# zjucsxxd/hdr2yuv

Measured on AMD Instinct MI355X. Metric: Mpixels/s, 4K RGB->YUV420 PQ convert path (in-memory, HBM-resident), higher is better.
Workload: dtype f32+f64

## Files before the change

hdr2yuv_amd/csrc/h2y_api.hip:

```cpp
#include <hip/hip_runtime.h>

#include <cstdarg>
#include <cstdio>
#include <cstdlib>
#include <algorithm>
#include <cstring>
#include <new>
#include <string>
#include <vector>

#include "../../include/hdr2yuv_hip.h"
#include "h2y_kernels.h"
#include "h2y_math.h"
#include "h2y_walk.h"

#include <zlib.h>

using namespace h2y;

namespace {

thread_local std::string g_err;

struct clip_limits {
// ... 79 lines not shown
    std::vector<double> bal_bwork;
    std::vector<uint32_t> range_slot[2];
    bool slot_busy[2] = {false, false};
    uint32_t *d_unit_rows = nullptr, *h_unit_rows = nullptr;
    size_t unit_rows_cap = 0;
    std::vector<uint32_t> dev_unit_rows;
    bool ffb_pending = false;
    double ffb_work[8] = {0, 0, 0, 0, 0, 0, 0, 0};
    frame_stats *d_fstats = nullptr, *h_fstats = nullptr;
    frame_stats *m_fstats = nullptr;
    frame_stats *fs_out = nullptr;
    assumed_stats *d_assumed = nullptr, *h_assumed = nullptr;
    assumed_stats dev_assumed;
    bool dev_assumed_ok = false;
    h2y_desc p_desc;
    int p_n = 0;
    bool p_check = false;
    bool was_t1 = false;
    std::vector<frame_io> p_frames;
    hipEvent_t ev_done = nullptr;
    hipEvent_t ev[kMaxEvents][2];
    int n_ev = 0;
};

struct h2y_ctx {
    int device = 0;
    batch_state bs[2];
    batch_state *b = &bs[0];
    int q_head = 0, q_count = 0;
    int n_cu = 0;
    hipStream_t own_stream = nullptr, stream = nullptr;
    hipStream_t fir_stream = nullptr;
    hipEvent_t ev_fused[2] = {nullptr, nullptr}, ev_fir[2] = {nullptr, nullptr};
    bool fir_used[2] = {false, false};
    void *d_table = nullptr;
    void *d_table1 = nullptr;
    void *d_table_ext = nullptr;
    void *d_tfn[H2Y_TFN_COUNT] = {};
    void *d_tfn_ext[H2Y_TFN_COUNT] = {};
    float *d_lut16 = nullptr;
    bool bal_have = false;
    double bal_speed[8] = {1, 1, 1, 1, 1, 1, 1, 1};
    std::vector<double> bal_bspeed;
    int bal_bgrid = 0, bal_bgroups = 0;
    bool ffb_have = false;
    double ffb_speed[8] = {1, 1, 1, 1, 1, 1, 1, 1};
    int t1_skip = 0, t1_skip_len = 0;
    bool cur_skip_t1 = false;
    bool opt_t1 = true;
    bool opt_t1_steer = true;
    int opt_groups = 0;
    bool opt_cols8 = true;
    int opt_bal_mode = 0;
    int opt_tail = 2;
    bool opt_bal_blocks = true;
    uint32_t opt_bal_mask = 0xFFu;
    double opt_bal_rho = 1.0;
    int opt_fir = 0;
    int opt_fir_sync = -1;
    double fir_flag_share = 0.0;
    uint16_t *d_tmp = nullptr;
    size_t tmp_cap = 0;
    uint16_t *d_lin = nullptr;
    void *d_tab = nullptr, *h_tab = nullptr;
    size_t d_tab_cap = 0, h_tab_cap = 0;
    cmp_partial *d_cmp_part = nullptr;
    size_t cmp_part_cap = 0;
    h2y_compare_stats *d_cmp_stats = nullptr;
    size_t cmp_stats_cap = 0;
    char *d_hist = nullptr;
    size_t hist_cap = 0;
    int64_t *d_ssim_part = nullptr;
    size_t ssim_part_cap = 0;
    h2y_ssim_stats *d_ssim_stats = nullptr;
    size_t ssim_stats_cap = 0;
    assumed_stats *d_light_as = nullptr;
    size_t light_as_cap = 0;
    light_acc *d_light_acc = nullptr;
    size_t light_acc_cap = 0;

    void *d_in = nullptr;
    size_t in_cap = 0;
    uint16_t *d_out = nullptr;
    size_t out_cap = 0;
    bool have_hint = false;
    int hint_kind = -1;
    int32_t hint_floor[3] = {0, 0, 0}, hint_ceil[3] = {0, 0, 0};
    struct stream_slot {
        char *h_in = nullptr;
        uint16_t *h_out = nullptr;
        char *d_in = nullptr;
        uint16_t *d_out = nullptr;
        hipEvent_t ev_h2d = nullptr, ev_conv = nullptr, ev_done = nullptr;
        int state = 0;
        char *h_ref = nullptr, *d_ref = nullptr;
        h2y_compare_stats *h_stats = nullptr;
        bool ref_lent = false;
        char *d_hist = nullptr;
        h2y_histogram_stats *h_hist_stats = nullptr;
        uint32_t *h_hist_bins = nullptr;
        h2y_ssim_stats *d_ssim = nullptr, *h_ssim = nullptr;
        light_acc *d_light = nullptr, *h_light = nullptr;
    };
    std::vector<stream_slot> ss;
    hipStream_t s_h2d = nullptr, s_d2h = nullptr;
    h2y_desc s_desc;
// ... 562 lines not shown
        for (int i = 0; i < nf; i++) {
            frame_io io = frames[f0 + i];
            if (out_kind == H2Y_OUT_444TMP) {
                io.tmp_cb = ctx->d_tmp + ((size_t)half * fir_sub + i) * tmp_stride;
                io.tmp_cr = io.tmp_cb + npix;
            } else if (yuvp2) {
                io.yuv = io.out;
                io.out = ctx->d_tmp + ((size_t)half * fir_sub + i) * tmp_stride;
                io.tmp_cr = nullptr;
            }
            const size_t idx = (size_t)ctx->slot_base + f0 + i;
            on_device = on_device && memcmp(&ctx->b->dev_frames[idx], &io, sizeof io) == 0;
            ctx->b->h_frames[idx] = io;
        }
        if (!on_device) {
            HIP_TRY(ctx, hipMemcpyAsync(ctx->b->d_frames + ctx->slot_base + f0, ctx->b->h_frames + ctx->slot_base + f0, nf * sizeof(frame_io), hipMemcpyHostToDevice,
                                        ctx->stream));
            for (int i = 0; i < nf; i++) ctx->b->dev_frames[(size_t)ctx->slot_base + f0 + i] = ctx->b->h_frames[(size_t)ctx->slot_base + f0 + i];
        }
        const int grid = grid_for(ctx, var, (uint64_t)g.chunks * nf);
        const int waves = h2y_fused_threads(var) / 64;
        int groups = 1;
        if (h2y_fused_grouped(var))
            for (int ng = groups_cap(ctx, g.tiles, grid); ng > 1; ng >>= 1)
                if (nf % ng == 0 && grid % ng == 0) {
                    groups = ng;
                    break;
                }
        if (nf / groups > kMaxFramesPerLaunch) return fail(ctx, H2Y_EINVAL, "internal: %d frames in %d groups exceed the per-group bound", nf, groups);
        int rc = ensure(ctx, ctx->b->d_partial, ctx->b->partial_cap, (size_t)nf * grid * waves * 6 * sizeof(float));
        if (rc) return rc;
        const bool t1 = var.pipe == 4 || var.pipe == 5;
        if (t1) {
            rc = ensure(ctx, ctx->b->d_redo, ctx->b->redo_cap, (size_t)nf * grid * waves * sizeof(uint32_t));
            if (rc) return rc;
        }
        const bool approx = var.pipe == 4;
        if (approx) {
            const size_t need = (size_t)(nf > 64 ? nf : 64) * sizeof(uint32_t);
            if (ctx->b->low_cap < need) {
                rc = ensure(ctx, ctx->b->d_low, ctx->b->low_cap, need);
                if (rc) return rc;
                HIP_TRY(ctx, hipMemsetAsync(ctx->b->d_low, 0, need, ctx->stream));
            }
        }
        if (check) ctx->b->approx_min = approx;
        const bool xcd_layout = h2y_fused_grouped(var) && grid % (8 * groups) == 0;
        const uint32_t *d_slice_ranges = nullptr;
        uint32_t range_stride = 0;
        bool tail_on = false;
        uint32_t tail_slices = 0;
        std::vector<double> bwork;
        double work[8] = {1, 1, 1, 1, 1, 1, 1, 1};
        if (xcd_layout && ctx->opt_bal_mode != 1) {
            const uint32_t G = (uint32_t)grid / (uint32_t)groups, nslices = (g.tiles + 63u) / 64u;
            double sp[8], mean = 0.0;
            for (int x = 0; x < 8; x++) {
                sp[x] = ctx->opt_bal_mode == 2 ? (((ctx->opt_bal_mask >> x) & 1u) ? ctx->opt_bal_rho : 1.0) : (ctx->bal_have ? ctx->bal_speed[x] : 1.0);
                mean += sp[x] / 8.0;
            }
            for (int x = 0; x < 8; x++) work[x] = sp[x] / mean;
            const bool per_block = ctx->opt_bal_mode == 0 && ctx->opt_bal_blocks && ctx->bal_bgrid == grid && ctx->bal_bgroups == groups &&
                                   (int)ctx->bal_bspeed.size() == grid && (size_t)groups * (G + 1u) <= kRangeWords;
            std::vector<uint32_t> r(per_block ? (size_t)groups * (G + 1u) : (size_t)G + 1u);
            bwork.assign((size_t)grid, 1.0);
            if (per_block) {
                std::vector<double> w(G);
                for (uint32_t gi = 0; gi < (uint32_t)groups; gi++) {
                    for (uint32_t i = 0; i < G; i++) w[i] = ctx->bal_bspeed[walk_block_of(gi, i, (uint32_t)groups)];
                    slice_ranges_w(w.data(), G, nslices, r.data() + (size_t)gi * (G + 1u));
                }
                range_stride = G + 1u;
            } else slice_ranges(sp, G, nslices, r.data());
            const int per_group = nf / groups;
            tail_on = t1 && ctx->opt_tail != 2 && nf % groups == 0 && per_group >= (ctx->opt_tail == 1 ? 2 : kTailMinFrames) && groups <= 16 &&

                      (uint64_t)(nslices / H2Y_TAIL_CHUNK + 96u) * 2u <= 64ull * G && G >= 8u;
            tail_slices = nslices;
            for (uint32_t gi = 0; gi < (uint32_t)groups; gi++) {
                const uint32_t *rg = r.data() + (size_t)(per_block ? gi : 0u) * (G + 1u);
                for (uint32_t i = 0; i < G; i++) bwork[walk_block_of(gi, i, (uint32_t)groups)] = (double)(rg[i + 1] - rg[i]) * (double)G / (double)nslices;
            }
            if (!ctx->b->h_ranges) {
                HIP_TRY(ctx, hipHostMalloc((void **)&ctx->b->h_ranges, 2 * kRangeWords * sizeof(uint32_t), hipHostMallocMapped));
                HIP_TRY(ctx, hipHostGetDevicePointer((void **)&ctx->b->hd_ranges, ctx->b->h_ranges, 0));
                HIP_TRY(ctx, hipHostMalloc((void **)&ctx->b->h_btime, 1024 * sizeof(float), hipHostMallocMapped));
                HIP_TRY(ctx, hipHostGetDevicePointer((void **)&ctx->b->hd_btime, ctx->b->h_btime, 0));
            }
            if (r.size() > kRangeWords) return fail(ctx, H2Y_EINVAL, "internal: %zu slice ranges", r.size());
            if (sub == 0 && !ctx->streaming) ctx->b->slot_busy[0] = ctx->b->slot_busy[1] = false;
            int slot = -1;
            for (int k = 0; k < 2 && slot < 0; k++)
                if (ctx->b->range_slot[k] == r) slot = k;
            if (slot < 0) {
                for (int k = 0; k < 2 && slot < 0; k++)
                    if (!ctx->b->slot_busy[k]) slot = k;
                if (slot < 0) {
                    HIP_TRY(ctx, hipStreamSynchronize(ctx->stream));
                    ctx->b->slot_busy[0] = ctx->b->slot_busy[1] = false;
                    slot = 0;
                }
                memcpy(ctx->b->h_ranges + (size_t)slot * kRangeWords, r.data(), r.size() * sizeof(uint32_t));
                ctx->b->range_slot[slot] = r;
            }
            ctx->b->slot_busy[slot] = true;
            d_slice_ranges = ctx->b->hd_ranges + (size_t)slot * kRangeWords;
        }
        const bool clocks = xcd_layout && time_it;
        if (clocks) {
            const size_t need = (size_t)2 * grid * sizeof(unsigned long long);
            if (ctx->b->clock_cap < need) {
                rc = ensure(ctx, ctx->b->d_clock, ctx->b->clock_cap, need);
                if (rc) return rc;
                HIP_TRY(ctx, hipMemsetAsync(ctx->b->d_clock, 0, need, ctx->stream));
            }
        }
        fused_args a;
        a.xcd_layout = xcd_layout ? 1u : 0u;
        a.block_clock = clocks ? ctx->b->d_clock : nullptr;
        a.slice_ranges = d_slice_ranges;
        a.range_stride = range_stride;
        a.tail_ctr = nullptr;
        a.tail_slices = 0;
        if (tail_on && d_slice_ranges) {
            if (!ctx->b->d_tail) {
                HIP_TRY(ctx, hipMalloc((void **)&ctx->b->d_tail, 16 * H2Y_TAIL_WORDS * sizeof(uint32_t)));
                HIP_TRY(ctx, hipMemsetAsync(ctx->b->d_tail, 0, 16 * H2Y_TAIL_WORDS * sizeof(uint32_t), ctx->stream));
            }
            a.tail_ctr = ctx->b->d_tail;
            a.tail_slices = tail_slices;
        }
        a.redo_count = t1 ? ctx->b->d_redo : nullptr;
        a.low_flag = approx ? ctx->b->d_low : nullptr;
        a.frames = ctx->b->d_frames + ctx->slot_base + f0;
        a.n_frames = nf;
        a.width = d->width;
        a.height = d->height;
        a.wq = g.wq;
        a.wq_magic = g.wq_magic;
        a.tiles_per_frame = g.tiles;
        a.chunks_per_frame = g.chunks;
        a.groups = (uint32_t)groups;
        a.table = ctx->d_table;
        a.table_src = a.table_dst = nullptr;
        a.lut16 = ctx->d_lut16;
        a.table1 = ctx->d_table1;
        a.sn = sn;
        a.partial = ctx->b->d_partial;
        a.assumed = d_assumed;
        a.pp = pp;
        if (pp.convert_transfer == 2 && !var.narrow && (var.pipe == 0 || var.pipe == 7)) {
            static const int kSrcFn[4] = {H2Y_TFN_NONE, H2Y_TFN_PQ_F, H2Y_TFN_RHO_H, H2Y_TFN_G24};
            static const int kDstFn[4] = {H2Y_TFN_NONE, H2Y_TFN_PQ_R, H2Y_TFN_RHO_R, H2Y_TFN_G24INV};
            const int sf = kSrcFn[pp.src_tf], df = kDstFn[pp.dst_tf];
            int rc2 = ensure_tfn(ctx, sf);
            if (!rc2) rc2 = ensure_tfn(ctx, df);
            if (rc2) return rc2;
            a.pp.src_fn = sf;
            a.pp.dst_fn = df;
            a.table_src = sf ? ctx->d_tfn[sf] : nullptr;
            a.table_dst = df ? ctx->d_tfn[df] : nullptr;
            a.pp.tf_ext[0] = sf ? ctx->d_tfn_ext[sf] : nullptr;
            a.pp.tf_ext[1] = df ? ctx->d_tfn_ext[df] : nullptr;
        }
        a.tiles_magic = g.tiles > 1 ? (uint32_t)(0x100000000ull / g.tiles) : 0xFFFFFFFFu;
        const bool ev = time_it && ctx->b->n_ev < kMaxEvents;
        if (ev) {
            HIP_TRY(ctx, hipEventRecord(ctx->b->ev[ctx->b->n_ev][0], ctx->stream));
            ctx->last_name = h2y_fused_name(var);
            static const char *const kIn[] = {"F32", "F16", "U16"}, *const kOut[] = {"420BOX", "444", "444TMP"};
            static const char *const kPipe[] = {"RUNTIME", "PQ_IDENT", "PQ_NORM", "LUT16", "PQ_IDENT", "PQ_NORM", "NONE", "TFN"};
            const char *mode = var.mode == H2Y_MODE_YCBCR ? "YCBCR" : var.mode == H2Y_MODE_YDZDX ? "YDZDX" : var.mode == H2Y_MODE_IDENTITY ? "IDENTITY"
                             : var.mode == H2Y_MODE_YUVP2 ? "YUVP2" : "YPQRS";
            char buf[192];
            snprintf(buf, sizeof buf, "%s<%s,%s,%s,%s%s>%s groups=%d xcd=%d%s", ctx->last_name, kIn[var.in_kind], kOut[var.out_kind], mode,
                     kPipe[var.pipe], var.cols8 ? ",COLS8" : "", out_kind == H2Y_OUT_444TMP ? "+k_fir420" : yuvp2 ? (d->chroma_resampler_type ? "+k_yuvp2_420<FIR>" : "+k_yuvp2_420<BOX>") : "", groups, xcd_layout ? 1 : 0,
                     a.tail_ctr ? " tail=1" : "");
            ctx->last_variant = buf;
        }
        HIP_TRY(ctx, h2y_launch_fused(var, grid, ctx->stream, a));
        if (ev) {
            HIP_TRY(ctx, hipEventRecord(ctx->b->ev[ctx->b->n_ev][1], ctx->stream));
            ctx->b->n_ev++;
        }
        final_args fa;
        fa.partial = ctx->b->d_partial;
        fa.nblk = grid / groups * waves;
        fa.redo_count = t1 ? ctx->b->d_redo : nullptr;
        fa.low_flag = approx ? ctx->b->d_low : nullptr;
        fa.out = ctx->b->fs_out + fstats_offset + f0;
        fa.is_u16 = d->in_sample_type == H2Y_SAMPLE_U16;
        fa.src_bit_depth = d->src_bit_depth;
        fa.check = check ? 1 : 0;
        fa.assumed = d_assumed;
        fa.publish = nullptr;
        fa.block_clock = clocks ? ctx->b->d_clock : nullptr;
        fa.grid = grid;
        static_assert(sizeof(frame_stats) >= 8 * sizeof(float), "the XCD run times ride in one frame_stats entry");
        fa.xcd_time = reinterpret_cast<float *>(ctx->b->fs_out + fstats_offset + n);
        fa.tail_ctr = a.tail_ctr;
        fa.tail_n = groups * (int)H2Y_TAIL_WORDS;
        fa.block_time = clocks && d_slice_ranges && ctx->b->fs_out == ctx->b->m_fstats ? ctx->b->hd_btime : nullptr;
        HIP_TRY(ctx, h2y_launch_stats_final(nf, ctx->stream, fa));
        if (clocks) {
            ctx->b->bal_slot = fstats_offset + n;
            ctx->b->bal_pending = true;
            for (int x = 0; x < 8; x++) ctx->b->bal_work[x] = work[x];
            ctx->b->bal_grid = fa.block_time ? grid : 0;
            ctx->b->bal_groups = groups;
            ctx->b->bal_bwork = bwork;
        }
        if (yuvp2) {
            HIP_TRY(ctx, hipEventRecord(ctx->ev_fused[half], ctx->stream));
            HIP_TRY(ctx, hipStreamWaitEvent(ctx->fir_stream, ctx->ev_fused[half], 0));
            yuvp2_args ya;
            ya.frames = ctx->b->d_frames + ctx->slot_base + f0;
            ya.n_frames = nf;
            ya.width = d->width;
            ya.height = d->height;
            ya.lin = ctx->d_lin;
            ya.fir_max = pp.fir_max;
            derive_params(d, &ya.pp, false);
            HIP_TRY(ctx, h2y_launch_yuvp2_420(d->chroma_resampler_type == 1, ctx->fir_stream, ya));
            HIP_TRY(ctx, hipEventRecord(ctx->ev_fir[half], ctx->fir_stream));
            ctx->fir_used[half] = true;
        }
        if (out_kind == H2Y_OUT_444TMP) {
            HIP_TRY(ctx, hipEventRecord(ctx->ev_fused[half], ctx->stream));
            HIP_TRY(ctx, hipStreamWaitEvent(ctx->fir_stream, ctx->ev_fused[half], 0));
            fir_args fr;
// ... 214 lines not shown
    if (e != hipSuccess || ndev < 1)
        return fail(nullptr, H2Y_EHIP, "no HIP device (%s): this library has no CPU path", hipGetErrorString(e));
    if (device < 0 || device >= ndev) return fail(nullptr, H2Y_EINVAL, "device %d out of range (have %d)", device, ndev);
    h2y_ctx *ctx = new (std::nothrow) h2y_ctx();
    if (!ctx) return fail(nullptr, H2Y_ENOMEM, "out of host memory");
    const int rc = ctx_init(ctx, device);
    if (rc) {
        h2y_ctx_destroy(ctx);
        return rc;
    }
    *out = ctx;
    return H2Y_OK;
}

int h2y_ctx_set_option(h2y_ctx *ctx, const char *name, const char *value)
{
    if (!ctx) return fail(nullptr, H2Y_EINVAL, "null ctx");
    if (!name || !value) return fail(ctx, H2Y_EINVAL, "null option name or value");
    if ((ctx->q_count > 0) || ctx->streaming) return fail(ctx, H2Y_EINVAL, "a batch is pending or a stream is open");
    if (!strcmp(name, "t1")) {
        ctx->opt_t1 = value[0] != '0';
        ctx->opt_t1_steer = strcmp(value, "always") != 0;
    }
    else if (!strcmp(name, "cols8")) ctx->opt_cols8 = value[0] != '0';
    else if (!strcmp(name, "firsync")) {
        int v = atoi(value), p = 1;
        if (!strcmp(value, "auto")) v = -1;
        else if (v < 0) return fail(ctx, H2Y_EINVAL, "firsync must be >= 0 or \"auto\"");
        while (2 * p <= v && p < 1024) p *= 2;
        ctx->opt_fir_sync = v > 0 ? p : v;
    } else if (!strcmp(name, "groups")) {
        int v = atoi(value), p = 1;
        if (v < 0) return fail(ctx, H2Y_EINVAL, "groups must be >= 0");
        while (2 * p <= v && p < 64) p *= 2;
        ctx->opt_groups = v ? p : 0;
    } else if (!strcmp(name, "balance")) {
        if (!strcmp(value, "adaptive")) { ctx->opt_bal_mode = 0; ctx->opt_bal_blocks = true; }
        else if (!strcmp(value, "xcd")) { ctx->opt_bal_mode = 0; ctx->opt_bal_blocks = false; }
        else if (!strcmp(value, "off")) ctx->opt_bal_mode = 1;
        else {
            char *end = nullptr;
            const unsigned long mm = strtoul(value, &end, 0);
            const double r = (end && *end == ',') ? atof(end + 1) : 0.0;
            if (!(mm & 0xFFu) || (mm & 0xFFu) == 0xFFu || !(r > 1.0)) return fail(ctx, H2Y_EINVAL, "balance: want adaptive, xcd, off or <mask>,<ratio > 1>");
            ctx->opt_bal_mode = 2;
            ctx->opt_bal_mask = (uint32_t)(mm & 0xFFu);
            ctx->opt_bal_rho = r;
        }
    } else if (!strcmp(name, "tail")) {
        if (!strcmp(value, "auto")) ctx->opt_tail = 0;
        else if (!strcmp(value, "on")) ctx->opt_tail = 1;
        else if (!strcmp(value, "off")) ctx->opt_tail = 2;
        else return fail(ctx, H2Y_EINVAL, "tail: want auto, on or off");
    } else if (!strcmp(name, "fir")) {
        if (!strcmp(value, "auto")) ctx->opt_fir = 0;
        else if (!strcmp(value, "twopass")) ctx->opt_fir = 1;
        else if (!strcmp(value, "fused")) ctx->opt_fir = 2;
        else return fail(ctx, H2Y_EINVAL, "fir: want auto, twopass or fused");
    } else return fail(ctx, H2Y_EINVAL, "unknown option '%s'", name);
    return H2Y_OK;
}

void h2y_ctx_destroy(h2y_ctx *ctx)
{
    if (!ctx) return;
    (void)hipSetDevice(ctx->device);
    if (ctx->stream) (void)hipStreamSynchronize(ctx->stream);
    if (ctx->streaming) (void)h2y_stream_close(ctx);
    for (batch_state &b : ctx->bs) {
        for (int i = 0; i < kMaxEvents; i++) {
            if (b.ev[i][0]) (void)hipEventDestroy(b.ev[i][0]);
            if (b.ev[i][1]) (void)hipEventDestroy(b.ev[i][1]);
        }
        if (b.ev_done) (void)hipEventDestroy(b.ev_done);
        (void)hipFree(b.d_frames);
        (void)hipHostFree(b.h_frames);
        (void)hipFree(b.d_partial);
        (void)hipFree(b.d_redo);
        (void)hipFree(b.d_low);
        (void)hipFree(b.d_clock);
        (void)hipHostFree(b.h_ranges);
        (void)hipHostFree(b.h_btime);
        (void)hipFree(b.d_tail);
        (void)hipFree(b.d_unit_rows);
        (void)hipHostFree(b.h_unit_rows);
        (void)hipFree(b.d_fstats);
        (void)hipHostFree(b.h_fstats);
        (void)hipFree(b.d_assumed);
        (void)hipHostFree(b.h_assumed);
    }
    (void)hipFree(ctx->d_table);
    for (void *t : ctx->d_tfn) (void)hipFree(t);
    for (int fn = 0; fn < H2Y_TFN_COUNT; fn++)
        if (ctx->d_tfn_ext[fn] && ctx->d_tfn_ext[fn] != ctx->d_table_ext) (void)hipFree(ctx->d_tfn_ext[fn]);
    (void)hipFree(ctx->d_lut16);
    (void)hipFree(ctx->d_table1);
    (void)hipFree(ctx->d_table_ext);
    (void)hipFree(ctx->d_tmp);
    (void)hipFree(ctx->d_lin);
    (void)hipFree(ctx->d_tab);
    (void)hipHostFree(ctx->h_tab);
    (void)hipFree(ctx->d_cmp_part);
    (void)hipFree(ctx->d_cmp_stats);
    (void)hipFree(ctx->d_hist);
    (void)hipFree(ctx->d_ssim_part);
    (void)hipFree(ctx->d_ssim_stats);
// ... 2564 lines not shown
```

hdr2yuv_amd/csrc/h2y_kernels.h:

```cpp
#ifndef H2Y_KERNELS_H
#define H2Y_KERNELS_H

#include <hip/hip_runtime.h>
#include <stdint.h>

#include "h2y_math.h"

#ifndef H2Y_FUSED_THREADS
#define H2Y_FUSED_THREADS 512
#endif
#ifndef H2Y_FUSED_MINWAVES
#define H2Y_FUSED_MINWAVES 4
#endif

#ifndef H2Y_LOOP_THREADS
#define H2Y_LOOP_THREADS 1024
#endif

#define H2Y_LUT16_N 16384

enum { H2Y_IN_F32 = 0, H2Y_IN_F16 = 1, H2Y_IN_U16 = 2 };
enum { H2Y_OUT_420BOX = 0, H2Y_OUT_444 = 1, H2Y_OUT_444TMP = 2 };

struct frame_io {
    const void *in[3];
    uint16_t *out;
    union {
        uint16_t *tmp_cb;
        uint16_t *yuv;
    };
    uint16_t *tmp_cr;
};

struct frame_stats {
    float mm[6];
    int32_t floor_[3];
    int32_t ceil_[3];
    int32_t mismatch;
    uint32_t redone;
};

struct assumed_stats {
    int32_t floor_[3];
    int32_t ceil_[3];
};

struct fused_args {
    const frame_io *frames;
    int n_frames;
    uint32_t width, height;
    uint32_t wq;
    uint32_t wq_magic;
    uint32_t tiles_per_frame;
    uint32_t chunks_per_frame;
    uint32_t groups;
    uint32_t xcd_layout;
    unsigned long long *block_clock;
    const uint32_t *slice_ranges;
    uint32_t *tail_ctr = nullptr;
    uint32_t tail_slices = 0;
    uint32_t range_stride = 0;
    const void *table;
    const void *table_src, *table_dst;
    const float *lut16;
    const void *table1;
    h2y::t1_sens sn;
    uint32_t tiles_magic;
    float *partial;
    uint32_t *redo_count;
    uint32_t *low_flag;
    const assumed_stats *assumed;
    h2y::pix_params pp;
};

struct fused_variant {
    int in_kind, out_kind, mode;
    int pipe;
    bool narrow;
    bool even_h;
    bool t1_ok = false;
    bool cols8 = false;
};

struct stats_args {
    const void *in[3];
    size_t npix;
    int vec_ok;
    float *partial;
};

struct final_args {
    const float *partial;
    const uint32_t *redo_count;
    uint32_t *low_flag;
    int nblk;
    frame_stats *out;
    int is_u16, src_bit_depth;
    int check;
    const assumed_stats *assumed;
    assumed_stats *publish;
    unsigned long long *block_clock;
    int grid;
    float *xcd_time;
    float *block_time = nullptr;
    uint32_t *tail_ctr = nullptr;
    int tail_n = 0;
};

struct fir_args {
    const frame_io *frames;
    int n_frames;
    const uint16_t *src_cb, *src_cr;
    uint16_t *dst_cb, *dst_cr;
// ... 197 lines not shown
```

hdr2yuv_amd/csrc/h2y_kernels.hip:

```cpp
#include <hip/hip_runtime.h>
#include <stdint.h>
#include <string.h>
#include <stdio.h>

#include "h2y_math.h"
#include "h2y_kernels.h"
#include "h2y_walk.h"
#include "h2y_device.h"

struct tile_pos {
    uint32_t tt;
    uint32_t q0, q1;
    bool row1;
};
__device__ __forceinline__ tile_pos tile_locate(uint32_t tt, uint32_t W, uint32_t H, uint32_t WQ, uint32_t magic)
{
    tile_pos t;
    uint32_t cg;
    (void)udiv_magic(tt, WQ, magic, cg);
    t.tt = tt;
    t.q0 = 2u * tt - cg;
    t.row1 = tt < WQ * (H >> 1);
    t.q1 = t.row1 ? t.q0 + WQ : t.q0;
    return t;
// ... 510 lines not shown
    const frame_io *frames;
    uint32_t *low_flag;
    uint32_t width, height, wq, wq_magic, tiles_per_frame, tiles_magic;
};
template <int IN_KIND, int OUT_KIND, int MODE, int PIPE>
__device__ __forceinline__ void redo_pass(const redo_ctx *rc, const pix_params *spp, const pq_recA *sA, const uint32_t *list,
                                                    uint32_t first, uint32_t cnt)
{
    const uint32_t lane = threadIdx.x & (WAVE - 1);
    if (lane >= cnt) return;
    const pq_recB *sB = reinterpret_cast<const pq_recB *>(sA + H2Y_PQ_NREC);
    uint32_t tt;
    const uint32_t f = udiv_magic(list[first + lane], rc->tiles_per_frame, rc->tiles_magic, tt);
    const frame_io io = rc->frames[f];
    const tile_pos t = tile_locate(tt, rc->width, rc->height, rc->wq, rc->wq_magic);
    tile_in v;
    tile_load<IN_KIND>(io, t, v);
    if (PIPE == H2Y_PIPE_PQ_IDENT && rc->low_flag) {
        float lo = min3f(min3f(v.g0[0], v.g0[1], v.g0[2]), min3f(v.g0[3], v.g1[0], v.g1[1]), min3f(v.g1[2], v.g1[3], v.b0[0]));
        lo = min3f(lo, min3f(v.b0[1], v.b0[2], v.b0[3]), min3f(v.b1[0], v.b1[1], v.b1[2]));
        lo = min3f(lo, min3f(v.b1[3], v.r0[0], v.r0[1]), min3f(v.r0[2], v.r0[3], v.r1[0]));
        lo = min3f(lo, min3f(v.r1[1], v.r1[2], v.r1[3]), lo);
        if (lo <= -1.0f) rc->low_flag[f] = 1u;
    }
    tile_out o;
    tile_exact<OUT_KIND, MODE, PIPE>(*spp, spp, sA, sB, v, o);
    tile_store<OUT_KIND>(io, t, rc->width, rc->height, o);
}

#ifdef H2Y_BLOCK_TIMES
__device__ unsigned long long g_block_times[2 * 1024];
void h2y_dump_block_times(const char *path)
{
    static unsigned long long h[2 * 1024];
    if (hipMemcpyFromSymbol(h, HIP_SYMBOL(g_block_times), sizeof h) != hipSuccess) return;
    FILE *f = fopen(path, "w");
    if (!f) return;
    for (int i = 0; i < 1024; i++) fprintf(f, "%d %llu %llu\n", i, h[2 * i], h[2 * i + 1]);
    fclose(f);
}
#endif
template <int IN_KIND, int OUT_KIND, int MODE, int PIPE>
__global__ __launch_bounds__(H2Y_T1_THREADS) void k_fused_t1(fused_args a)
{
#ifdef H2Y_BLOCK_TIMES
    if (threadIdx.x == 0) g_block_times[2 * blockIdx.x] = wall_clock64();
#endif
    __shared__ pq_rec1 s_t1[H2Y_T1_NREC];
    __shared__ pq_recA s_t2[2 * H2Y_PQ_NREC];
    __shared__ uint32_t s_redo[H2Y_T1_THREADS / WAVE][H2Y_REDO_CAP];
    __shared__ pix_params s_pp;
    __shared__ redo_ctx s_rc;
    __shared__ uint32_t s_claim[H2Y_CLAIM_FRAMES], s_scratch[WAVE];
    __shared__ uint32_t s_tq[H2Y_TAIL_QLEN + 3], s_tbounds[1];
    {
        stage16<H2Y_T1_THREADS, H2Y_T1_NREC>(a.table1, s_t1);
        stage_table<H2Y_T1_THREADS>(a.table, s_t2);
        if (threadIdx.x < H2Y_CLAIM_FRAMES) s_claim[threadIdx.x] = 0u;
        if (threadIdx.x < H2Y_TAIL_QLEN) s_tq[threadIdx.x] = 0xFFFFFFFFu;
        if (threadIdx.x == 0) {
            s_tq[H2Y_TAIL_QLEN] = (blockIdx.x * 37u) & (H2Y_TAIL_PARTS - 1u);
            s_tq[H2Y_TAIL_QLEN + 1] = 0u;
            s_tq[H2Y_TAIL_QLEN + 2] = 0u;
        }
        if (a.tail_ctr && threadIdx.x == 0) s_tbounds[0] = a.tail_slices;
    }
    const pix_params pp = with_assumed(a.pp, a.assumed);
    t1_sens sn = a.sn;
    asm volatile("" : "+v"(sn.a_lo), "+v"(sn.a_hi));
    if (threadIdx.x == 0) {
        s_pp = pp;
        s_rc.frames = a.frames;
        s_rc.low_flag = a.low_flag;
        s_rc.width = a.width; s_rc.height = a.height; s_rc.wq = a.wq; s_rc.wq_magic = a.wq_magic;
        s_rc.tiles_per_frame = a.tiles_per_frame; s_rc.tiles_magic = a.tiles_magic;
    }
    __syncthreads();
    __shared__ uint32_t s_black[3];
    if (threadIdx.x == 0) {
        const pq_recB *sB2 = reinterpret_cast<const pq_recB *>(s_t2 + H2Y_PQ_NREC);
        const float G0 = norm1<PIPE>(pp, 0, 0.0f), B0 = norm1<PIPE>(pp, 1, 0.0f), R0 = norm1<PIPE>(pp, 2, 0.0f);
        uint32_t y, cb, cr;
        if (pixel_fast<MODE, PIPE>(pp, s_t2, sB2, G0, B0, R0, y, cb, cr)) {
            const ycc k = pixel_careful<MODE>(&s_pp, G0, B0, R0);
            y = k.y; cb = k.cb; cr = k.cr;
        }
        s_black[0] = y; s_black[1] = cb - pp.half_m1; s_black[2] = cr - pp.half_m1;
    }
    __syncthreads();

    block_clock_start(a);
    const uint32_t W = a.width, H = a.height;
    const uint32_t lane = threadIdx.x & (WAVE - 1), wave = threadIdx.x / WAVE;
    const pq_recB *const sB2 = reinterpret_cast<const pq_recB *>(s_t2 + H2Y_PQ_NREC);
    uint32_t *const my_list = s_redo[wave];
    uint32_t n_redo = 0;
    tile_in v;
    tile_pos t_cur;
    bool have = false;
    typedef in_traits<IN_KIND> IN;
    frame_walk fw;
    uint32_t fo = 0;
    uint32_t tick = 0;
    bool hold = false;
    uint32_t dyn_carry = 0, dyn_t0_next = 0;
    walk_init(fw, a);
    typedef const __attribute__((address_space(4))) fused_args *args_ptr;
    args_ptr ap = (args_ptr)__builtin_amdgcn_kernarg_segment_ptr();
    const uint32_t grp = (uint32_t)fw.f;
    uint32_t r_first, r_count;
    const bool ranged = block_range(a, fw, r_first, r_count);
    constexpr uint32_t kTqNone = 0xFFFFFFFFu, kTqEmpty = 0xFFFFFFFEu;
    volatile uint32_t *const tq = s_tq;
    uint32_t *const tail_ctr = a.tail_ctr ? a.tail_ctr + grp * H2Y_TAIL_WORDS : nullptr;
    auto draw_chunk = [&](uint32_t c) {
        tail_state ts;
        ts.part = tq[H2Y_TAIL_QLEN];
        ts.tried = tq[H2Y_TAIL_QLEN + 1];
        const uint32_t n_slices = s_tbounds[0];
        uint32_t got = kTqEmpty;
        uint32_t known[2] = {0u, 0u};
        while (!ts.done()) {
            if ((known[ts.part >> 5] >> (ts.part & 31u)) & 1u) { ts.skip(); continue; }
            uint32_t cv = 0u;
            if (lane == 0) cv = __hip_atomic_fetch_add(tail_ctr + ts.part, 1u, __ATOMIC_RELAXED, __HIP_MEMORY_SCOPE_AGENT);
            uint32_t first, count;
            if (ts.take(n_slices, __builtin_amdgcn_readfirstlane(cv), &first, &count)) {
                got = first | (count << 24);
                break;
            }
            uint32_t k0 = 0u, k1 = 0u;
            if (lane == 0) {
                k0 = __hip_atomic_fetch_or(tail_ctr + H2Y_TAIL_PARTS + (ts.part >> 5), 1u << (ts.part & 31u), __ATOMIC_RELAXED, __HIP_MEMORY_SCOPE_AGENT);
                k1 = __hip_atomic_load(tail_ctr + H2Y_TAIL_PARTS + ((ts.part >> 5) ^ 1u), __ATOMIC_RELAXED, __HIP_MEMORY_SCOPE_AGENT);
            }
            known[ts.part >> 5] = __builtin_amdgcn_readfirstlane(k0) | (1u << (ts.part & 31u));
            known[(ts.part >> 5) ^ 1u] = __builtin_amdgcn_readfirstlane(k1);
            ts.skip();
        }
        if (lane == 0) {
            tq[H2Y_TAIL_QLEN] = ts.part;
            tq[H2Y_TAIL_QLEN + 1] = ts.tried;
            asm volatile("" ::: "memory");
            tq[c] = got;
        }
    };
    auto dyn_tile0 = [&](uint32_t tk, uint32_t &tile0) -> bool {
        const uint32_t c = tk / H2Y_TAIL_CHUNK, idx = tk % H2Y_TAIL_CHUNK;
        if (c >= H2Y_TAIL_QLEN) return false;
        if (tk == 0u) draw_chunk(0u);
        uint32_t e;
        while ((e = tq[c]) == kTqNone) __builtin_amdgcn_s_sleep(1);
        asm volatile("" ::: "memory");
        if (idx == 0u && c + 1u < H2Y_TAIL_QLEN) {
            if (e == kTqEmpty) { if (lane == 0) tq[c + 1u] = kTqEmpty; }
            else draw_chunk(c + 1u);
        }
        if (e == kTqEmpty) return false;
        const uint32_t cnt = e >> 24;
        tile0 = ((e & 0xFFFFFFu) + (idx < cnt ? idx : cnt - 1u)) * WAVE;
        return true;
    };
    for (; fw.f < fw.n_frames; fw.advance(), fo++) {
        const int f = fw.f;
        const bool dyn = tail_ctr != nullptr && !fw.has_next();
        const bool dyn_n = tail_ctr != nullptr && fw.has_next() && f + 2 * (int)fw.NG >= fw.n_frames;
        uint32_t dyn_t0 = 0;
        asm volatile("" : "+s"(ap));
        const frame_io *const frames = ap->frames;
        const frame_io io = uniform_io(frames + f);
        typedef const __attribute__((address_space(4))) frame_io *frame_cptr;
        const frame_cptr io_next_p = (frame_cptr)(uintptr_t)(frames + (fw.has_next() ? f + (int)fw.NG : f));
        mm6 mm;
        mm.reset();
        const uint32_t id_base = (uint32_t)f * a.tiles_per_frame;
        uint32_t flagged_f = 0;
        uint32_t flagged_px = 0;
        wave_deal deal, deal_n;
        if (ranged) {
            deal.set_range(r_first, r_count);
            deal_n.set_range(r_first, r_count);
        } else {
            deal.set(fw, fw.k0, H2Y_T1_THREADS / WAVE);
            deal_n.set(fw, fw.k0_n, H2Y_T1_THREADS / WAVE);
        }
        if (dyn) {
            if (!hold) {
                tick = wave_claim(&s_tq[H2Y_TAIL_QLEN + 2], s_scratch, true);
                hold = dyn_tile0(tick, dyn_t0);
            } else dyn_t0 = dyn_carry;
        } else if (!hold) {
            tick = wave_claim(&s_claim[fo], s_scratch, true);
            hold = tick < deal.total;
        }
        bool more = hold;
        while (more) {
            if (!have) {
                t_cur = tile_locate(umin32((dyn ? dyn_t0 : deal.tile0<H2Y_T1_THREADS>(tick)) + lane, a.tiles_per_frame - 1u), W, H, a.wq, a.wq_magic);
                tile_load<IN_KIND>(io, t_cur, v);
            }
#pragma unroll
            for (int j = 0; j < 4; j++)
                asm volatile("" ::"v"(v.g0[j]), "v"(v.b0[j]), "v"(v.r0[j]), "v"(v.g1[j]), "v"(v.b1[j]), "v"(v.r1[j]));
            do {
                const uint32_t tt = (dyn ? dyn_t0 : deal.tile0<H2Y_T1_THREADS>(tick)) + lane;
                tile_pos t = t_cur;
                t.row1 = true;
                const void *src[3];
                int kind;
                uint32_t tick2;
                tile_pos t2;
                const uint32_t n1v = wave_claim_issue(dyn ? &s_tq[H2Y_TAIL_QLEN + 2] : &s_claim[fo], s_scratch);

                tile_in nx;
                {
                        {
                            const uint32_t n1 = __builtin_amdgcn_readfirstlane(n1v);
                            uint32_t tt2;
                            if (__builtin_expect(dyn, 0)) {
                                uint32_t t0n = 0;
                                const bool same = dyn_tile0(n1, t0n);
                                kind = same ? 1 : 0;
                                tick2 = same ? n1 : tick;
                                tt2 = same ? t0n : dyn_t0;
                                dyn_t0_next = tt2;
                            } else {
                            const bool same = n1 < deal.total;
                            if (__builtin_expect(same, 1)) {
                                kind = 1;
                                tick2 = n1;
                                tt2 = deal.tile0<H2Y_T1_THREADS>(n1);
                            } else {
                                const bool try_next = fw.has_next();
                                bool nextf;
                                uint32_t n2, t0n = 0;
                                if (dyn_n) {
                                    n2 = wave_claim(&s_tq[H2Y_TAIL_QLEN + 2], s_scratch, true);
                                    nextf = dyn_tile0(n2, t0n);
                                    dyn_carry = t0n;
                                } else {
                                    n2 = wave_claim(&s_claim[(fo + 1u) & (H2Y_CLAIM_FRAMES - 1u)], s_scratch, try_next);
                                    nextf = try_next && n2 < deal_n.total;
                                    if (nextf) t0n = deal_n.tile0<H2Y_T1_THREADS>(n2);
                                }
                                kind = nextf ? 2 : 0;
                                tick2 = nextf ? n2 : tick;
                                tt2 = nextf ? t0n : deal.tile0<H2Y_T1_THREADS>(tick);
                            }
                            }
                            kind = __builtin_amdgcn_readfirstlane(kind);
                            tick2 = __builtin_amdgcn_readfirstlane(tick2);
                            tt2 = __builtin_amdgcn_readfirstlane(tt2);
                            hold = have = kind != 0;
#pragma unroll
                            for (int c = 0; c < 3; c++) src[c] = io.in[c];
                            if (__builtin_expect(kind == 2, 0)) {
#pragma unroll
                                for (int c = 0; c < 3; c++) src[c] = io_next_p->in[c];
                            }
                            t2 = tile_locate(umin32(tt2 + lane, a.tiles_per_frame - 1u), W, H, a.wq, a.wq_magic);
                        }
                    IN::load4q(src[0], t2.q0, nx.g0);
                    IN::load4q(src[1], t2.q0, nx.b0);
                    IN::load4q(src[2], t2.q0, nx.r0);
                    IN::load4q(src[0], t2.q1, nx.g1);
                    IN::load4q(src[1], t2.q1, nx.b1);
                    IN::load4q(src[2], t2.q1, nx.r1);
                    __builtin_amdgcn_sched_barrier(0);
                }
                tile_out o;
                uint32_t sb[2], sr[2];
                uint64_t redo_m = 0;
#pragma unroll
                for (int row = 0; row < 2; row++) {
                    const float(&gv)[4] = row ? v.g1 : v.g0;
                    const float(&bv)[4] = row ? v.b1 : v.b0;
                    const float(&rv)[4] = row ? v.r1 : v.r0;
#ifdef H2Y_EXP_NOSTATS
                    if (false) {
#else
                    if (PIPE == H2Y_PIPE_PQ_IDENT) {
#endif
                        if (row == 0) { mm.add2(0, gv[0], gv[1]); mm.add2(1, bv[0], bv[1]); mm.add2(2, rv[0], rv[1]); }
                        else { mm.add2_max(0, gv[0], gv[1]); mm.add2_max(1, bv[0], bv[1]); mm.add2_max(2, rv[0], rv[1]); }
                        mm.add2_max(0, gv[2], gv[3]); mm.add2_max(1, bv[2], bv[3]); mm.add2_max(2, rv[2], rv[3]);
                    } else {
#ifndef H2Y_EXP_NOSTATS
                        mm.add2(0, gv[0], gv[1]); mm.add2(0, gv[2], gv[3]);
                        mm.add2(1, bv[0], bv[1]); mm.add2(1, bv[2], bv[3]);
                        mm.add2(2, rv[0], rv[1]); mm.add2(2, rv[2], rv[3]);
#endif
                    }
                    uint32_t Y[4], Cb[4], Cr[4];
                    bool zrow = false;
                    if (__builtin_expect(__builtin_amdgcn_ballot_w64(f2bits(gv[0]) != 0u) == 0, 0)) {
                        const uint32_t z = (f2bits(gv[1]) | f2bits(gv[2]) | f2bits(gv[3])) | (f2bits(bv[0]) | f2bits(bv[1]) | f2bits(bv[2])) |
                                           (f2bits(bv[3]) | f2bits(rv[0]) | f2bits(rv[1])) | (f2bits(rv[2]) | f2bits(rv[3]));
                        zrow = __builtin_amdgcn_ballot_w64(z != 0u) == 0;
                    }
                    if (zrow) {
                        const uint32_t y0 = s_black[0], cb0 = s_black[1], cr0 = s_black[2];
#pragma unroll
                        for (int col = 0; col < 4; col++) { Y[col] = y0; Cb[col] = cb0; Cr[col] = cr0; }
                    } else
#pragma unroll
                    for (int col = 0; col < 4; col++) {
#ifdef H2Y_EXP_NOCOMPUTE
                        Y[col] = f2bits(gv[col]) >> 20; Cb[col] = f2bits(bv[col]) >> 20; Cr[col] = f2bits(rv[col]) >> 20;
                        continue;
#endif
#ifdef H2Y_HALF_COMPUTE
// ... 798 lines not shown
```

hdr2yuv_amd/csrc/h2y_walk.h:

```cpp
#ifndef H2Y_WALK_H
#define H2Y_WALK_H
#include "h2y_math.h"

namespace h2y {

struct walk_args {
    uint32_t groups, xcd_layout, chunks_per_frame;
    int n_frames;
};

struct frame_walk {
    uint32_t G, NG, bi;
    uint32_t cpf, mod, gb;
    int f, n_frames;
    uint32_t k0, k0_n;

    H2Y_FN uint32_t wrap(uint32_t x) const { return x >= G ? x - G : x; }
    H2Y_FN void set_firsts()
    {
        k0 = wrap(bi + G - gb);
        k0_n = wrap(bi + G - wrap(gb + mod));
    }
    H2Y_FN void init(const walk_args &a, uint32_t b , uint32_t grid )
    {
// ... 33 lines not shown
        return same ? 1 : next ? 2 : 0;
    }
    H2Y_FN uint32_t count(uint32_t k) const { return k < cpf ? (cpf - 1u - k) / G + 1u : 0u; }
    H2Y_FN size_t slot() const { return (size_t)f * G + bi; }
};

inline void slice_ranges_w(const double *w , uint32_t G, uint32_t n_slices, uint32_t *r)
{
    double tot = 0.0;
    for (uint32_t i = 0; i < G; i++) tot += w[i];
    double cum = 0.0;
    for (uint32_t i = 0; i <= G; i++) {
        r[i] = i == G ? n_slices : (uint32_t)(cum / tot * (double)n_slices + 0.5);
        if (i < G) cum += w[i];
    }
}
inline void slice_ranges(const double speed[8], uint32_t G, uint32_t n_slices, uint32_t *r)
{
    double w[1024];
    for (uint32_t i = 0; i < G && i < 1024u; i++) w[i] = speed[i % 8u];
    slice_ranges_w(w, G, n_slices, r);
}
H2Y_FN uint32_t walk_block_of(uint32_t g, uint32_t i, uint32_t NG) { return (((i >> 3) * NG + g) << 3) | (i & 7u); }

#define H2Y_TAIL_CHUNK 32u
#define H2Y_TAIL_PARTS 64u
#define H2Y_TAIL_WORDS (H2Y_TAIL_PARTS + 2u)
struct tail_state {
    uint32_t part, tried;
    H2Y_FN void init(uint32_t start) { part = start & (H2Y_TAIL_PARTS - 1u); tried = 0; }
    H2Y_FN bool done() const { return tried >= H2Y_TAIL_PARTS; }
    H2Y_FN void range(uint32_t n_slices, uint32_t *lo, uint32_t *hi) const
    {
        *lo = (uint32_t)(((uint64_t)n_slices * part) / H2Y_TAIL_PARTS);
        *hi = (uint32_t)(((uint64_t)n_slices * (part + 1u)) / H2Y_TAIL_PARTS);
    }
    H2Y_FN void skip()
    {
        tried++;
        part = (part + 1u) & (H2Y_TAIL_PARTS - 1u);
    }
    H2Y_FN bool take(uint32_t n_slices, uint32_t c, uint32_t *first, uint32_t *count) const
    {
        uint32_t lo, hi;
        range(n_slices, &lo, &hi);
        const uint64_t start = (uint64_t)lo + (uint64_t)c * H2Y_TAIL_CHUNK;
        if (start >= hi) return false;
        *first = (uint32_t)start;
        *count = hi - (uint32_t)start < H2Y_TAIL_CHUNK ? hi - (uint32_t)start : H2Y_TAIL_CHUNK;
        return true;
    }
};

}
#endif
```

Baseline: 378,600.

## Add dynamic sweep dealing of tile chunks across all frames per group

Adds a 'deal' option where blocks claim 64-slice chunks from a global atomic counter that sweeps through every frame of a group, replacing static per-block slice ranges and per-frame claims when the tail option is off (the default). The shared tail queue becomes a ring buffer tagged with chunk index and frame, so a wave can jump across frames while prefetching its next tile. The goal is to remove load imbalance between blocks and XCDs across the whole launch, not only in the last frame. The cost is a global atomic per chunk, more shared-memory bookkeeping, and the loss of the measured per-XCD balancing path and block clocks.

```diff
diff --git a/hdr2yuv_amd/csrc/h2y_api.hip b/hdr2yuv_amd/csrc/h2y_api.hip
--- a/hdr2yuv_amd/csrc/h2y_api.hip
+++ b/hdr2yuv_amd/csrc/h2y_api.hip
@@ -155,6 +155,7 @@
     int opt_groups = 0;
     bool opt_cols8 = true;
     int opt_bal_mode = 0;
+    int opt_deal = 0;
     int opt_tail = 2;
     bool opt_bal_blocks = true;
     uint32_t opt_bal_mask = 0xFFu;
@@ -823,7 +824,10 @@
         uint32_t tail_slices = 0;
         std::vector<double> bwork;
         double work[8] = {1, 1, 1, 1, 1, 1, 1, 1};
-        if (xcd_layout && ctx->opt_bal_mode != 1) {
+        const uint32_t frame_slices = (g.tiles + 63u) / 64u;
+        const bool sweep = t1 && (ctx->opt_deal == 1 || (ctx->opt_deal == 0 && ctx->opt_tail == 2)) && groups <= 16 && nf % groups == 0 &&
+                           frame_slices < (1u << 24);
+        if (xcd_layout && ctx->opt_bal_mode != 1 && !sweep) {
             const uint32_t G = (uint32_t)grid / (uint32_t)groups, nslices = (g.tiles + 63u) / 64u;
             double sp[8], mean = 0.0;
             for (int x = 0; x < 8; x++) {
@@ -877,7 +881,7 @@
             ctx->b->slot_busy[slot] = true;
             d_slice_ranges = ctx->b->hd_ranges + (size_t)slot * kRangeWords;
         }
-        const bool clocks = xcd_layout && time_it;
+        const bool clocks = xcd_layout && time_it && !sweep;
         if (clocks) {
             const size_t need = (size_t)2 * grid * sizeof(unsigned long long);
             if (ctx->b->clock_cap < need) {
@@ -893,13 +897,15 @@
         a.range_stride = range_stride;
         a.tail_ctr = nullptr;
         a.tail_slices = 0;
-        if (tail_on && d_slice_ranges) {
+        a.sweep = 0;
+        if ((tail_on && d_slice_ranges) || sweep) {
             if (!ctx->b->d_tail) {
                 HIP_TRY(ctx, hipMalloc((void **)&ctx->b->d_tail, 16 * H2Y_TAIL_WORDS * sizeof(uint32_t)));
                 HIP_TRY(ctx, hipMemsetAsync(ctx->b->d_tail, 0, 16 * H2Y_TAIL_WORDS * sizeof(uint32_t), ctx->stream));
             }
             a.tail_ctr = ctx->b->d_tail;
-            a.tail_slices = tail_slices;
+            a.tail_slices = sweep ? frame_slices : tail_slices;
+            a.sweep = sweep ? 1u : 0u;
         }
         a.redo_count = t1 ? ctx->b->d_redo : nullptr;
         a.low_flag = approx ? ctx->b->d_low : nullptr;
@@ -946,7 +952,7 @@
             char buf[192];
             snprintf(buf, sizeof buf, "%s<%s,%s,%s,%s%s>%s groups=%d xcd=%d%s", ctx->last_name, kIn[var.in_kind], kOut[var.out_kind], mode,
                      kPipe[var.pipe], var.cols8 ? ",COLS8" : "", out_kind == H2Y_OUT_444TMP ? "+k_fir420" : yuvp2 ? (d->chroma_resampler_type ? "+k_yuvp2_420<FIR>" : "+k_yuvp2_420<BOX>") : "", groups, xcd_layout ? 1 : 0,
-                     a.tail_ctr ? " tail=1" : "");
+                     a.sweep ? " deal=dyn" : a.tail_ctr ? " tail=1" : "");
             ctx->last_variant = buf;
         }
         HIP_TRY(ctx, h2y_launch_fused(var, grid, ctx->stream, a));
@@ -1267,6 +1273,11 @@
         else if (!strcmp(value, "on")) ctx->opt_tail = 1;
         else if (!strcmp(value, "off")) ctx->opt_tail = 2;
         else return fail(ctx, H2Y_EINVAL, "tail: want auto, on or off");
+    } else if (!strcmp(name, "deal")) {
+        if (!strcmp(value, "dynamic")) ctx->opt_deal = 1;
+        else if (!strcmp(value, "static")) ctx->opt_deal = 2;
+        else if (!strcmp(value, "auto")) ctx->opt_deal = 0;
+        else return fail(ctx, H2Y_EINVAL, "deal: want dynamic, static or auto");
     } else if (!strcmp(name, "fir")) {
         if (!strcmp(value, "auto")) ctx->opt_fir = 0;
         else if (!strcmp(value, "twopass")) ctx->opt_fir = 1;
diff --git a/hdr2yuv_amd/csrc/h2y_kernels.h b/hdr2yuv_amd/csrc/h2y_kernels.h
--- a/hdr2yuv_amd/csrc/h2y_kernels.h
+++ b/hdr2yuv_amd/csrc/h2y_kernels.h
@@ -59,6 +59,7 @@
     const uint32_t *slice_ranges;
     uint32_t *tail_ctr = nullptr;
     uint32_t tail_slices = 0;
+    uint32_t sweep = 0;
     uint32_t range_stride = 0;
     const void *table;
     const void *table_src, *table_dst;
diff --git a/hdr2yuv_amd/csrc/h2y_kernels.hip b/hdr2yuv_amd/csrc/h2y_kernels.hip
--- a/hdr2yuv_amd/csrc/h2y_kernels.hip
+++ b/hdr2yuv_amd/csrc/h2y_kernels.hip
@@ -586,18 +586,27 @@
     __shared__ pix_params s_pp;
     __shared__ redo_ctx s_rc;
     __shared__ uint32_t s_claim[H2Y_CLAIM_FRAMES], s_scratch[WAVE];
-    __shared__ uint32_t s_tq[H2Y_TAIL_QLEN + 3], s_tbounds[1];
+    __shared__ uint32_t s_tq[H2Y_TAIL_QLEN + 3], s_tqtag[H2Y_TAIL_QLEN], s_tqfr[H2Y_TAIL_QLEN], s_tbounds[4];
     {
         stage16<H2Y_T1_THREADS, H2Y_T1_NREC>(a.table1, s_t1);
         stage_table<H2Y_T1_THREADS>(a.table, s_t2);
         if (threadIdx.x < H2Y_CLAIM_FRAMES) s_claim[threadIdx.x] = 0u;
-        if (threadIdx.x < H2Y_TAIL_QLEN) s_tq[threadIdx.x] = 0xFFFFFFFFu;
+        if (threadIdx.x < H2Y_TAIL_QLEN) s_tqtag[threadIdx.x] = 0xFFFFFFFFu;
         if (threadIdx.x == 0) {
             s_tq[H2Y_TAIL_QLEN] = (blockIdx.x * 37u) & (H2Y_TAIL_PARTS - 1u);
             s_tq[H2Y_TAIL_QLEN + 1] = 0u;
             s_tq[H2Y_TAIL_QLEN + 2] = 0u;
         }
-        if (a.tail_ctr && threadIdx.x == 0) s_tbounds[0] = a.tail_slices;
+        if (a.tail_ctr && threadIdx.x == 0) {
+            frame_walk w0;
+            walk_init(w0, a);
+            sweep_deal sd;
+            sd.init(a.tail_slices, ((uint32_t)a.n_frames - (uint32_t)w0.f + a.groups - 1u) / a.groups);
+            s_tbounds[0] = a.tail_slices;
+            s_tbounds[1] = a.sweep ? sd.cpf : 0u;
+            s_tbounds[2] = sd.n_chunks;
+            s_tbounds[3] = (uint32_t)(a.n_frames - 1 - w0.f) / a.groups;
+        }
     }
     const pix_params pp = with_assumed(a.pp, a.assumed);
     t1_sens sn = a.sn;
@@ -638,21 +647,34 @@
     uint32_t tick = 0;
     bool hold = false;
     uint32_t dyn_carry = 0, dyn_t0_next = 0;
+    uint32_t dyn_fr = 0;
+    bool dyn_done = false;
     walk_init(fw, a);
     typedef const __attribute__((address_space(4))) fused_args *args_ptr;
     args_ptr ap = (args_ptr)__builtin_amdgcn_kernarg_segment_ptr();
     const uint32_t grp = (uint32_t)fw.f;
     uint32_t r_first, r_count;
     const bool ranged = block_range(a, fw, r_first, r_count);
-    constexpr uint32_t kTqNone = 0xFFFFFFFFu, kTqEmpty = 0xFFFFFFFEu;
+    constexpr uint32_t kTqEmpty = 0xFFFFFFFEu;
     volatile uint32_t *const tq = s_tq;
     uint32_t *const tail_ctr = a.tail_ctr ? a.tail_ctr + grp * H2Y_TAIL_WORDS : nullptr;
+    volatile uint32_t *const tqtag = s_tqtag, *const tqfr = s_tqfr;
     auto draw_chunk = [&](uint32_t c) {
+        uint32_t got = kTqEmpty, fr = s_tbounds[3];
+        if (s_tbounds[1]) {
+            sweep_deal sd;
+            sd.n_slices = s_tbounds[0];
+            sd.cpf = s_tbounds[1];
+            sd.n_chunks = s_tbounds[2];
+            uint32_t k = 0u;
+            if (lane == 0) k = __hip_atomic_fetch_add(tail_ctr, 1u, __ATOMIC_RELAXED, __HIP_MEMORY_SCOPE_AGENT);
+            uint32_t first, count;
+            if (sd.take(__builtin_amdgcn_readfirstlane(k), &fr, &first, &count)) got = first | (count << 24);
+        } else {
         tail_state ts;
         ts.part = tq[H2Y_TAIL_QLEN];
         ts.tried = tq[H2Y_TAIL_QLEN + 1];
         const uint32_t n_slices = s_tbounds[0];
-        uint32_t got = kTqEmpty;
         uint32_t known[2] = {0u, 0u};
         while (!ts.done()) {
             if ((known[ts.part >> 5] >> (ts.part & 31u)) & 1u) { ts.skip(); continue; }
@@ -675,20 +697,34 @@
         if (lane == 0) {
             tq[H2Y_TAIL_QLEN] = ts.part;
             tq[H2Y_TAIL_QLEN + 1] = ts.tried;
+        }
+        }
+        if (lane == 0) {
+            const uint32_t slot = c & (H2Y_TAIL_QLEN - 1u);
+            tq[slot] = got;
+            tqfr[slot] = fr;
             asm volatile("" ::: "memory");
-            tq[c] = got;
+            tqtag[slot] = c;
         }
     };
-    auto dyn_tile0 = [&](uint32_t tk, uint32_t &tile0) -> bool {
-        const uint32_t c = tk / H2Y_TAIL_CHUNK, idx = tk % H2Y_TAIL_CHUNK;
-        if (c >= H2Y_TAIL_QLEN) return false;
+    static_assert(H2Y_TAIL_CHUNK == 32u && H2Y_SWEEP_CHUNK == 64u, "chunk sizes as shifts below");
+    const uint32_t tq_shift = a.sweep ? 6u : 5u;
+    auto dyn_tile0 = [&](uint32_t tk, uint32_t &tile0, uint32_t &fr) -> bool {
+        const uint32_t c = tk >> tq_shift, idx = tk & ((1u << tq_shift) - 1u), slot = c & (H2Y_TAIL_QLEN - 1u);
         if (tk == 0u) draw_chunk(0u);
-        uint32_t e;
-        while ((e = tq[c]) == kTqNone) __builtin_amdgcn_s_sleep(1);
+        while (tqtag[slot] != c) __builtin_amdgcn_s_sleep(1);
         asm volatile("" ::: "memory");
-        if (idx == 0u && c + 1u < H2Y_TAIL_QLEN) {
-            if (e == kTqEmpty) { if (lane == 0) tq[c + 1u] = kTqEmpty; }
-            else draw_chunk(c + 1u);
+        const uint32_t e = tq[slot];
+        fr = __builtin_amdgcn_readfirstlane(tqfr[slot]);
+        if (idx == 0u) {
+            if (e == kTqEmpty) {
+                if (lane == 0) {
+                    const uint32_t s1 = (c + 1u) & (H2Y_TAIL_QLEN - 1u);
+                    tq[s1] = kTqEmpty;
+                    asm volatile("" ::: "memory");
+                    tqtag[s1] = c + 1u;
+                }
+            } else draw_chunk(c + 1u);
         }
         if (e == kTqEmpty) return false;
         const uint32_t cnt = e >> 24;
@@ -697,8 +733,9 @@
     };
     for (; fw.f < fw.n_frames; fw.advance(), fo++) {
         const int f = fw.f;
-        const bool dyn = tail_ctr != nullptr && !fw.has_next();
-        const bool dyn_n = tail_ctr != nullptr && fw.has_next() && f + 2 * (int)fw.NG >= fw.n_frames;
+        const bool sweep = tail_ctr != nullptr && ap->sweep != 0u;
+        const bool dyn = tail_ctr != nullptr && (sweep || !fw.has_next());
+        const bool dyn_n = tail_ctr != nullptr && !sweep && fw.has_next() && f + 2 * (int)fw.NG >= fw.n_frames;
         uint32_t dyn_t0 = 0;
         asm volatile("" : "+s"(ap));
         const frame_io *const frames = ap->frames;
@@ -719,15 +756,17 @@
             deal_n.set(fw, fw.k0_n, H2Y_T1_THREADS / WAVE);
         }
         if (dyn) {
-            if (!hold) {
+            if (!hold && !dyn_done) {
                 tick = wave_claim(&s_tq[H2Y_TAIL_QLEN + 2], s_scratch, true);
-                hold = dyn_tile0(tick, dyn_t0);
-            } else dyn_t0 = dyn_carry;
+                hold = dyn_tile0(tick, dyn_carry, dyn_fr);
+                dyn_done = !hold;
+            }
+            dyn_t0 = dyn_carry;
         } else if (!hold) {
             tick = wave_claim(&s_claim[fo], s_scratch, true);
             hold = tick < deal.total;
         }
-        bool more = hold;
+        bool more = hold && (!dyn || dyn_fr == fo);
         while (more) {
             if (!have) {
                 t_cur = tile_locate(umin32((dyn ? dyn_t0 : deal.tile0<H2Y_T1_THREADS>(tick)) + lane, a.tiles_per_frame - 1u), W, H, a.wq, a.wq_magic);
@@ -742,7 +781,7 @@
                 t.row1 = true;
                 const void *src[3];
                 int kind;
-                uint32_t tick2;
+                uint32_t tick2, nskip = 0;
                 tile_pos t2;
                 const uint32_t n1v = wave_claim_issue(dyn ? &s_tq[H2Y_TAIL_QLEN + 2] : &s_claim[fo], s_scratch);
 
@@ -752,12 +791,17 @@
                             const uint32_t n1 = __builtin_amdgcn_readfirstlane(n1v);
                             uint32_t tt2;
                             if (__builtin_expect(dyn, 0)) {
-                                uint32_t t0n = 0;
-                                const bool same = dyn_tile0(n1, t0n);
-                                kind = same ? 1 : 0;
-                                tick2 = same ? n1 : tick;
-                                tt2 = same ? t0n : dyn_t0;
+                                uint32_t t0n = 0, frn = 0;
+                                const bool got = dyn_tile0(n1, t0n, frn);
+                                const bool same = got && frn == fo;
+                                kind = same ? 1 : got ? 2 : 0;
+                                tick2 = got ? n1 : tick;
+                                tt2 = got ? t0n : dyn_t0;
+                                nskip = got && !same ? frn - fo - 1u : 0u;
                                 dyn_t0_next = tt2;
+                                dyn_carry = t0n;
+                                dyn_fr = frn;
+                                dyn_done = !got;
                             } else {
                             const bool same = n1 < deal.total;
                             if (__builtin_expect(same, 1)) {
@@ -770,7 +814,7 @@
                                 uint32_t n2, t0n = 0;
                                 if (dyn_n) {
                                     n2 = wave_claim(&s_tq[H2Y_TAIL_QLEN + 2], s_scratch, true);
-                                    nextf = dyn_tile0(n2, t0n);
+                                    nextf = dyn_tile0(n2, t0n, dyn_fr);
                                     dyn_carry = t0n;
                                 } else {
                                     n2 = wave_claim(&s_claim[(fo + 1u) & (H2Y_CLAIM_FRAMES - 1u)], s_scratch, try_next);
@@ -785,12 +829,13 @@
                             kind = __builtin_amdgcn_readfirstlane(kind);
                             tick2 = __builtin_amdgcn_readfirstlane(tick2);
                             tt2 = __builtin_amdgcn_readfirstlane(tt2);
+                            nskip = __builtin_amdgcn_readfirstlane(nskip);
                             hold = have = kind != 0;
 #pragma unroll
                             for (int c = 0; c < 3; c++) src[c] = io.in[c];
                             if (__builtin_expect(kind == 2, 0)) {
 #pragma unroll
-                                for (int c = 0; c < 3; c++) src[c] = io_next_p->in[c];
+                                for (int c = 0; c < 3; c++) src[c] = io_next_p[nskip * fw.NG].in[c];
                             }
                             t2 = tile_locate(umin32(tt2 + lane, a.tiles_per_frame - 1u), W, H, a.wq, a.wq_magic);
                         }
diff --git a/hdr2yuv_amd/csrc/h2y_walk.h b/hdr2yuv_amd/csrc/h2y_walk.h
--- a/hdr2yuv_amd/csrc/h2y_walk.h
+++ b/hdr2yuv_amd/csrc/h2y_walk.h
@@ -109,5 +109,24 @@
     }
 };
 
+#define H2Y_SWEEP_CHUNK 64u
+struct sweep_deal {
+    uint32_t n_slices, cpf, n_chunks;
+    H2Y_FN void init(uint32_t slices_per_frame, uint32_t group_frames)
+    {
+        n_slices = slices_per_frame;
+        cpf = (slices_per_frame + H2Y_SWEEP_CHUNK - 1u) / H2Y_SWEEP_CHUNK;
+        n_chunks = cpf * group_frames;
+    }
+    H2Y_FN bool take(uint32_t k, uint32_t *frame, uint32_t *first, uint32_t *count) const
+    {
+        if (k >= n_chunks) return false;
+        *frame = k / cpf;
+        *first = (k - *frame * cpf) * H2Y_SWEEP_CHUNK;
+        *count = n_slices - *first < H2Y_SWEEP_CHUNK ? n_slices - *first : H2Y_SWEEP_CHUNK;
+        return true;
+    }
+};
+
 }
 #endif
```

New measurement: 374,300 (median of 2 runs). -1.1%, worse.
